# TrevorS/voxtral-mini-realtime-rs

Measured on AMD Instinct MI355X. Metric: decode_tok_per_s, higher is better.
Workload: dtype f32

## Files before the change

### voxtral-mini-realtime-rs_amd/csrc/vox_api.cpp

```cpp
#include "../../include/voxtral_hip.h"
#include "vox_kernels.h"

#include <dlfcn.h>
#include <fcntl.h>
#include <sys/mman.h>
#include <sys/stat.h>
#include <unistd.h>

#include <algorithm>
#include <chrono>
#include <cmath>
#include <cstdarg>
#include <cstdio>
#include <cstdlib>
#include <cstring>
#include <map>
#include <mutex>
#include <string>
#include <unordered_map>
#include <thread>
#include <vector>

using namespace vox;

// ... 661 lines not shown
static std::mutex g_cache_mu; static std::unordered_map<const vox_cache*, uint64_t> g_cache_live; static uint64_t g_cache_gen = 0;
static void cache_register(vox_cache* k) { std::lock_guard<std::mutex> l(g_cache_mu); k->gen = ++g_cache_gen; g_cache_live[k] = k->gen; }
static void cache_unregister(const vox_cache* k) { std::lock_guard<std::mutex> l(g_cache_mu); g_cache_live.erase(k); }
static bool cache_alive(const vox_cache* k, uint64_t gen) { std::lock_guard<std::mutex> l(g_cache_mu); auto it = g_cache_live.find(k); return it != g_cache_live.end() && it->second == gen; }

struct TensorMeta { std::vector<uint64_t> shape; int dtype = 0; uint64_t nbytes = 0; };
struct vox_model {
    vox_ctx* ctx = nullptr; vox_model_cfg cfg{};
    std::vector<vox_model*> twins;
    std::map<std::string, TensorMeta> manifest; bool is_q4 = false;
    uint8_t* arena = nullptr; uint64_t arena_bytes = 0, arena_primary_bytes = 0;
    std::vector<Q4W*> tiled;
    const float *conv1_w = nullptr, *conv1_b = nullptr, *conv2_w = nullptr, *conv2_b = nullptr, *enc_norm = nullptr, *dec_norm = nullptr;
    Q4W conv1_g{}, conv2_g{};
    const float *enc_cos = nullptr, *enc_sin = nullptr, *dec_cos = nullptr, *dec_sin = nullptr;
    int enc_rope_len = 4096, dec_rope_len = 16384;
    std::vector<EncLayer> enc; std::vector<DecLayer> dec; Lin ad0, ad2, tok;
    float* ada_mul = nullptr; bool t_embed_set = false; std::vector<float> t_embed_host;
    float* ws = nullptr; size_t ws_floats = 0;
    float *d_audio = nullptr; int audio_cap = 0;
    float *d_mel = nullptr; size_t mel_cap = 0;
    float *d_samples = nullptr; size_t samples_cap = 0;
    vox_cache* cache = nullptr;
    int *d_tokens = nullptr, *d_pos = nullptr; int tokens_cap = 0;
    float* d_prefix = nullptr;
    float *enc_cos_s = nullptr, *enc_sin_s = nullptr; int enc_rope_s_len = 0;
    int* d_seq_len = nullptr; std::vector<int> h_seq_len;
    int *d_seq_off = nullptr, *d_row_pos = nullptr; size_t row_pos_cap = 0; std::vector<int> h_seq_off, h_row_pos;
    float *d_h = nullptr, *d_q = nullptr, *d_att = nullptr, *d_act = nullptr, *d_logits = nullptr, *d_part_val = nullptr; int* d_part_idx = nullptr;
    float* d_h2 = nullptr; long long* d_wo_acc = nullptr;
    int n_parts = 0, argmax_R = 8;
    bool eng_ok = false, eng_on = true, eng_ready = false; unsigned char* eng_stream = nullptr; unsigned char* eng_state = nullptr; EngLayerTab* eng_tab = nullptr;
    const vox_cache* eng_tab_cache = nullptr; const float* eng_tab_k = nullptr; std::vector<EngLayerTab> eng_tab_host;
    int eng_flags = 128 | 512 | 1, eng_pace = 50;
    unsigned long long eng_launches = 0; unsigned eng_err_host[2] = {0, 0};
    int eng_strikes = 0; bool eng_suspended = false;
    unsigned char* eng_wob = nullptr;
    bool engb_ok = false; unsigned char* engb_state[4] = {nullptr, nullptr, nullptr, nullptr}; EngLayerTab* engb_tab[4] = {nullptr, nullptr, nullptr, nullptr};
    bool engb_on = true; unsigned long long engb_launches = 0; int engb_strikes = 0;
    int batch_sessions = 0;
    int engb_flags = 128 | 1 | 64 | 2048;
    int engb_flags2 = 128 | 1024;
    unsigned engb_err_host[4][2] = {{0, 0}, {0, 0}, {0, 0}, {0, 0}};
    hipGraph_t graph[2] = {nullptr, nullptr}; hipGraphExec_t graph_exec[2] = {nullptr, nullptr}; int graph_unroll = 0, graph_mode = 0;
    const vox_cache* graph_cache = nullptr; const float* graph_audio = nullptr;
    float *pw_x = nullptr, *pw_hidden = nullptr, *pw_logits = nullptr; size_t pw_x_cap = 0, pw_hidden_cap = 0, pw_logits_cap = 0;
    float* pw_part_val = nullptr; int* pw_part_idx = nullptr; int* pw_ids = nullptr; int pw_ids_cap = 0; int* pw_zero = nullptr;
    EngLayerTab* pw_tab = nullptr; const vox_cache* pw_tab_cache = nullptr; uint64_t pw_tab_gen = 0;
    bool pw_memo = false, pw_eng_used = false;
    vox_cache* pw_pend_cache = nullptr; uint64_t pw_pend_gen = 0; int pw_pend_rows = 0; bool pw_verdict_failed = false;
    unsigned* pw_err_pin = nullptr;
    vox_timings timings{};
};

struct Arena {
    uint8_t* base = nullptr; uint64_t off = 0;
    template <class T> T* take(size_t count) {
        off = (off + 255) / 256 * 256;
        T* p = base ? reinterpret_cast<T*>(base + off) : nullptr;
        off += count * sizeof(T);
        return p;
    }
};

#define ENC_PFX "mm_streams_embeddings.embedding_module.whisper_encoder"
#define EMB_PFX "mm_streams_embeddings.embedding_module"
#define TOK_NAME EMB_PFX ".tok_embeddings.weight"
// ... 2553 lines not shown
```

### voxtral-mini-realtime-rs_amd/csrc/vox_engine.hip

```cpp
#include "vox_kernels.h"

#include <hip/hip_fp16.h>

#include <cstdio>
#include <cstdlib>

namespace vox {
namespace {

#include "vox_engine_common.h"

__global__ __launch_bounds__(64) void eng_pack_lm_kernel(Q4W w, unsigned char* __restrict__ stream, size_t op_off, int vocab) {
    const int q = blockIdx.x, b = blockIdx.y, lane = threadIdx.x;
    const int row = lm_rows_per_cu(vocab) * b + q;
    unsigned char* dst = stream + (size_t)NCU * (op_off + (size_t)(q / NCONS) * PK_A) + (size_t)b * PK_A + (size_t)(q % NCONS) * PASS_A;
    const size_t src = (size_t)row * w.nb + lane;
    reinterpret_cast<uint4*>(dst)[lane] = w.qs[src];
    reinterpret_cast<uint16_t*>(dst + PA_S0)[lane] = w.sc[src];
    const size_t sh = (size_t)row * w.nb + 64 + (lane >> 1);
    const uint4 qh = w.qs[sh];
    reinterpret_cast<uint2*>(dst + PA_Q1)[lane] = (lane & 1) ? make_uint2(qh.z, qh.w) : make_uint2(qh.x, qh.y);
    if ((lane & 1) == 0) reinterpret_cast<uint16_t*>(dst + PA_S1)[lane >> 1] = w.sc[sh];
}
__global__ __launch_bounds__(64) void eng_pack_kernel(Q4W w, int op, unsigned char* __restrict__ stream, size_t op_off) {
    const int pk = blockIdx.x / (NCONS * 4), wv = (blockIdx.x / 4) % NCONS, s = blockIdx.x % 4, b = blockIdx.y, lane = threadIdx.x, n = lane & 15, g = lane >> 4;
    const int steps = pk_steps(op, pk); const bool half = pk_half_tile(op, pk);
    if (s >= steps || (half && n >= 8)) return;
    int tile, T; rec_src(op, pk, wv, s, &tile, &T);
    const int row = tile_row(op, b, tile, n), blk0 = step_blk0(op, b, T);
    const size_t pk_bytes = (size_t)op_pk_bytes(op), rec_bytes = half ? REC_H : REC;
    unsigned char* dst = stream + (size_t)NCU * (op_off + (size_t)pk * pk_bytes) + (size_t)b * pk_bytes + (size_t)wv * steps * rec_bytes + (size_t)s * rec_bytes;
    const uint4 q = w.qs[(size_t)row * w.nb + blk0 + (g >> 1)];
    reinterpret_cast<uint2*>(dst)[half ? g * 8 + n : lane] = (g & 1) ? make_uint2(q.z, q.w) : make_uint2(q.x, q.y);
    if (g < 2) reinterpret_cast<uint16_t*>(dst + (half ? REC_H_SC : REC_SC))[(half ? 8 : 16) * g + n] = w.sc[(size_t)row * w.nb + blk0 + g];
}

struct EngCtl {
    unsigned ring_ready[8], ring_done[8];
    unsigned xs0_flag, xs1_flag, xa_flag, qkv_flag;
    unsigned cbar, dead, gathering, gw_flag;
    unsigned xcd_ok, xcc_id, ag_flag, pub_cnt;
    float rstd0, rstd1, pad1, pad2;
    float best_val[16]; int best_idx[16];
    float h_own[16], h1_own[16];
    unsigned ag_done, pad_q[3];
    float rope_c[24], rope_s[24];
};
constexpr int L_RING = 0;
constexpr int L_XS = L_RING + NSLOT * SLOT_BYTES;
constexpr int L_U = L_XS + ED * 4;
constexpr int L_XA = L_U;
constexpr int L_PART = L_U;
constexpr int L_SC = L_U;
constexpr int L_PO = L_SC + SC_MAX * 4;
constexpr int L_PL = L_PO + 12 * 128 * 4;
constexpr int L_QKVN = L_PL + 64;
constexpr int L_TMP = L_QKVN + 384 * 4;
constexpr int L_SSQ = L_TMP + 384 * 4;
constexpr int L_BLK = L_SSQ + NCU * 4;
constexpr int L_TAB = L_BLK + 96 * 8;
constexpr int MAX_LAYERS = 32;
constexpr int L_GW = L_TAB + MAX_LAYERS * (int)sizeof(EngLayerTab);
constexpr int L_CTL = L_GW + (MAX_LAYERS + 1) * 32 * 4;
constexpr int L_TOTAL = L_CTL + (int)sizeof(EngCtl);
static_assert(L_TOTAL <= 160 * 1024, "LDS budget");
static_assert(L_TAB % 16 == 0 && sizeof(EngLayerTab) == 40, "layer table");
static_assert(L_XS % 16 == 0 && L_XA % 16 == 0 && L_QKVN % 16 == 0 && L_PO % 16 == 0 && L_CTL % 16 == 0 && L_BLK % 8 == 0 && 72 * 12 * 4 <= SC_MAX * 4 && 1152 * 4 + 96 * 6 * 4 <= SC_MAX * 4 + 12 * 128 * 4, "aligned carve");

__device__ __forceinline__ void eng_loader(const EngParams& p, EngCtl* c, unsigned ring_lds, int lane, const Tl& tl) {
    Loader<EngCtl, NSLOT> ld; ld.c = c; ld.err = p.err; ld.ring_lds = ring_lds; ld.voff = (unsigned)lane * 16u; ld.thin = (p.flags & 1) != 0; ld.pace = (u64)p.pace_ticks;
    const bool fake = (p.flags & 2) != 0;
    const bool nodma = (p.flags & 32) != 0;
    if (p.flags & 64) ld.pause_ticks = 300;
    if (p.flags & 1024) ld.depth = 2;
    if (p.flags & 2048) ld.depth = 1;
    const u64 base = (u64)p.stream;
    const unsigned n_layer_pk = (unsigned)p.n_layers * PK_LAYER, n_pk = n_layer_pk + (unsigned)lm_packets(p.vocab);
    unsigned l = 0, r = 0;
    u64 off = 0;
#pragma unroll 1
    for (unsigned pk = 0; pk < n_pk; pk++) {
        int bytes = PK_A;
        if (pk < n_layer_pk) {
            if (r < PK_LAYER_M) bytes = PK_M;
            if (r == 0 && (int)l == p.tl_layer) tl(16);
        } else { ld.pace = 0; ld.pause_ticks = 0; ld.depth = 3; }
        const u64 src = fake ? base + (u64)blockIdx.x * PK_A : base + (u64)NCU * off + (u64)blockIdx.x * (u64)bytes;
        if (bytes == PK_M) ld.issue<PK_M>(src, lane, nodma); else ld.issue<PK_A>(src, lane, nodma);
        off += (u64)bytes;
        if (++r == PK_LAYER) { if ((int)l == p.tl_layer) tl(17); r = 0; l++; }
    }
    ld.flush();
    tl(18);
}


__device__ __forceinline__ void comm_probe_x(const EngParams& p, EngCtl* c, int lane, const u64* src, unsigned tag, const Tl& tl, bool T) {
    const srd_t sd = make_srd(src, ED * 8u);
    if (T) tl(20);
    u64 t0 = 0;
    if (p.flags & 512) {
        const u64 tw = wall_clock64();
        while (wall_clock64() - tw < (u64)p.ag_delay_ticks) __builtin_amdgcn_s_sleep(1);
    } else
    for (;;) {
        const u64 gq = ld_gran(sd, 48u * (unsigned)lane);
        if (__all((unsigned)(gq >> 32) == tag)) break;
        if (sweep_bail(t0, tag, c, p.err)) break;
    }
    if (T) tl(21);
}
__device__ __forceinline__ void comm_publish_rows(const EngParams& p, int lane, float hraw, float gw, u64* dst, u64* ssq, unsigned tag, float* own) {
    const int b = blockIdx.x;
    float sq = lane < OWN ? hraw * hraw : 0.f;
    sq = row16_sum_e(sq);
    if (lane < OWN) { publish(dst + OWN * b + lane, tag, hraw * gw); own[lane] = hraw; }
    if (lane == 0) publish(ssq + b, tag, sq);
}

// ... 18 lines not shown
    const unsigned c = own_k >> 5, e = own_k & 31;
    const size_t blk = (size_t)token * (size_t)p.tok_nb + c;
    const unsigned byte = ((const __attribute__((address_space(1))) unsigned char*)(uintptr_t)p.tok_qs)[blk * 16 + (e & 15)];
    const float d = __half2float(__ushort_as_half(((const __attribute__((address_space(1))) unsigned short*)(uintptr_t)p.tok_sc)[blk]));
    const int nib = e < 16 ? (int)(byte & 15u) : (int)(byte >> 4);
    return __fadd_rn(au, __fmul_rn(__fsub_rn((float)nib, 8.0f), d));
}

__device__ __forceinline__ void eng_comm(const EngParams& p, EngCtl* c, unsigned char* lds, const int lane0, const Tl& tl) {
    const int b = blockIdx.x, g = b & 7, j = b >> 3, h = 4 * g + (j >> 3);
    float* xa = reinterpret_cast<float*>(lds + L_XA); float* qkvn = reinterpret_cast<float*>(lds + L_QKVN);
    float* tmp = reinterpret_cast<float*>(lds + L_TMP);
    const EngLayerTab* tab = reinterpret_cast<const EngLayerTab*>(lds + L_TAB);
    const unsigned tag_base = (*p.serial + 1u) * 64u;
    const bool PROBE_SMALL = (p.flags & 4) != 0;
    const int own_r = min(lane0, OWN - 1);
    const unsigned own_k = (unsigned)(OWN * b + own_r);
    const float* gwt = reinterpret_cast<const float*>(lds + L_GW);
    {
        const float g0 = ld_gf(make_srd(p.n_layers > 0 ? tab[0].attn_norm : p.final_norm, ED * 4u), own_k) * (p.n_layers > 0 ? 1.0f : 512.0f);
        const float hraw = (p.flags & ENGF_ARGMAX_IN) ? comm_next_input(p, lane0, own_k) : ld_gf(make_srd(p.h_in, ED * 4u), own_k);
        comm_publish_rows(p, lane0, hraw, g0, p.H0, p.SS0, tag_base, c->h_own);
    }
#pragma unroll 1
    for (int st = 0; st <= 2 * p.n_layers; st++) {
        int lane = lane0; asm volatile("" : "+v"(lane));
        const int l = st >> 1; const bool odd = st & 1, last = st == 2 * p.n_layers, T = l == p.tl_layer;
        const unsigned tag = tag_base + (unsigned)l + 1u;
        if (odd) comm_probe_x(p, c, lane, p.H1, tag, tl, T);
        else comm_probe_x(p, c, lane, p.H0, tag - 1u, tl, false);
        lds_st(&c->gathering, 1u);
        lds_st(&c->ag_flag, (unsigned)st + 1u);
        if (T) tl(odd ? 11 : 8);
        if (p.flags & (1 | 64)) wait_ge(&c->ag_done, NCONS * ((unsigned)st + 1u), c, p.err, ERR_STAGE);
        lds_st(&c->gathering, 0u);
        if (last) break;
        if (!odd) {
            wait_ge(&c->gw_flag, (unsigned)NCONS, c, p.err, ERR_STAGE);
            const bool xloc_nt = (p.flags & 128) != 0 && (p.flags & 4096) != 0 && lds_ld(&c->xcd_ok) != 0;
            {
                wait_ge(&c->pub_cnt, NCONS * (4u * (unsigned)l + 1u), c, p.err, ERR_STAGE);
                lds_st(&c->gathering, 1u);
                float v[6];
                sweep<6>(p.G, (EQD + 2 * EKD) * 8u, tag, [&](int u) { const int i = lane + 64 * u, seg = i >> 7, e = i & 127; return seg == 0 ? 128 * h + e : (seg == 1 ? EQD : EQD + EKD) + 128 * g + e; },
                         [&]() { return lane < 32 ? EQD + 128 * g + 4 * lane : EQD + EKD + 128 * g + 4 * (lane - 32); }, PROBE_SMALL, v, c, p.err, xloc_nt);
                lds_st(&c->gathering, 0u);
#pragma unroll
                for (int u = 0; u < 6; u++) qkvn[lane + 64 * u] = v[u];
                ENG_CFENCE(); lds_st(&c->qkv_flag, (unsigned)l + 1u);
            }
            if (T) tl(9);
            {
                wait_ge(&c->pub_cnt, NCONS * (4u * (unsigned)l + 2u), c, p.err, ERR_STAGE);
                lds_st(&c->gathering, 1u);
                float v[6];
                sweep<6>(p.PW, NPW * ED * 8u, tag, [&](int u) { const int i = lane + 64 * u, hh = i / OWN, r = i - hh * OWN; return hh * ED + OWN * b + r; }, [&]() { return (lane & 31) * ED + OWN * b; }, PROBE_SMALL, v, c, p.err);
#pragma unroll
                for (int u = 0; u < 6; u++) tmp[lane + 64 * u] = v[u];
                lds_st(&c->gathering, 0u);
                ENG_CFENCE();
                float a = 0.f;
                const int r = min(lane, OWN - 1);
#pragma unroll 4
                for (int hh = 0; hh < NPW; hh++) a += tmp[hh * OWN + r];
                wait_ge(&c->gw_flag, (unsigned)NCONS, c, p.err, ERR_STAGE);
                if (!((p.flags & 16384) && blockIdx.x == 7 && l == 1))
                    comm_publish_rows(p, lane, c->h_own[r] + a, gwt[(l * 2 + 1) * 16 + r], p.H1, p.SS1, tag, c->h1_own);
// ... 132 lines not shown
    e = max(e, -100);
    const float f = ldexpf(1.0f, 26 - e);
    int xi[4];
#pragma unroll
    for (int i = 0; i < 4; i++) xi[i] = (int)rintf(v[i] * f);
    int s = (xi[0] + xi[1]) + (xi[2] + xi[3]);
    s += dppi<0xB1>(s); s += dppi<0x4E>(s); s += dppi<0x141>(s);
    if ((lane & 7) == 0) *binfo_blk = make_float2(-8.0f * (float)s, ldexpf(1.0f, e - 26));
    const int e0 = 4 * (lane & 7), h = (e0 >> 3) & 1, off = (e0 & 4) + 8 * (e0 >> 4);
#pragma unroll
    for (int cdig = 0; cdig < 4; cdig++) {
        unsigned d = 0;
#pragma unroll
        for (int i = 0; i < 4; i++) { const int dv = cdig < 3 ? (xi[i] >> (7 * cdig)) & 127 : xi[i] >> 21; d |= (unsigned)(dv & 0xFF) << (8 * i); }
        *reinterpret_cast<unsigned*>(plane_blk + (cdig * 2 + h) * 16 + off) = d;
    }
}

struct Cons {
    const EngParams& p; EngCtl* c; unsigned char* lds; int cw, lane; unsigned P; unsigned cbar_n;
    __device__ __forceinline__ Cons(const EngParams& p_, EngCtl* c_, unsigned char* lds_, int cw_, int lane_) : p(p_), c(c_), lds(lds_), cw(cw_), lane(lane_), P(0), cbar_n(0) {}
    __device__ __forceinline__ void cbarrier() {
        cbar_n += NCONS;
        ENG_CFENCE();
        if (lane == 0) __hip_atomic_fetch_add(&c->cbar, 1u, RLX, WG);
        wait_ge(&c->cbar, cbar_n, c, p.err, ERR_CBAR);
    }
    __device__ __forceinline__ void published(const Tl& tl, int evt) {
        ENG_CFENCE();
        if (lane == 0) { const unsigned old = __hip_atomic_fetch_add(&c->pub_cnt, 1u, RLX, WG); if (evt >= 0 && tl.buf && old % NCONS == NCONS - 1) tl.buf[evt] = wall_clock64(); }
    }
    __device__ __forceinline__ const unsigned char* slot_wait(unsigned pk, int share_bytes, int& slot) {
        slot = (int)(pk % NSLOT); const unsigned k = pk / NSLOT;
        wait_ge(&c->ring_ready[slot], k + 1u, c, p.err, ERR_RING);
        return lds + L_RING + slot * SLOT_BYTES + cw * share_bytes;
    }
    __device__ __forceinline__ void slot_release(int slot) {
        ENG_CFENCE();
        if (lane == 0) __hip_atomic_fetch_add(&c->ring_done[slot], 1u, RLX, WG);
    }
    __device__ __forceinline__ void fetch(unsigned pk, PassA& P_) {
        int slot; const unsigned char* base = slot_wait(pk, PASS_A, slot);
        P_.q0 = reinterpret_cast<const uint4*>(base)[lane];
        P_.q1 = reinterpret_cast<const uint2*>(base + PA_Q1)[lane];
        P_.s0 = __half2float(__ushort_as_half(reinterpret_cast<const unsigned short*>(base + PA_S0)[lane]));
        P_.s1 = __half2float(__ushort_as_half(reinterpret_cast<const unsigned short*>(base + PA_S1)[lane >> 1]));
        slot_release(slot);
    }
    static __device__ __forceinline__ float dot(const PassA& P_, const XA& xr) { return fmaf(P_.s1, half_dot(P_.q1, xr.xh, xr.m8h), P_.s0 * block_dot(P_.q0, xr.x, xr.m8)); }

    template <bool DIGITS>
    __device__ __forceinline__ float all_gather(const u64* src, const u64* ssq, unsigned tag, unsigned stage, unsigned char* xs, float* ssl, float2* binfo, const Tl& tl, bool T) {
        wait_ge(&c->ag_flag, stage + 1u, c, p.err, ERR_STAGE);
        const srd_t sd = make_srd(src, ED * 8u), qd = make_srd(ssq, NCU * 8u);
        int ln = lane; asm volatile("" : "+v"(ln));
        if (DIGITS) {
            const unsigned q = 64u * (unsigned)cw + (unsigned)ln;
            u32x4 ra, rb; u64 rq = 0, t0 = 0;
            for (;;) {
                ra = __builtin_bit_cast(u32x4, __builtin_amdgcn_raw_buffer_load_b128(sd, (int)(q * 32u), 0, 16));
                rb = __builtin_bit_cast(u32x4, __builtin_amdgcn_raw_buffer_load_b128(sd, (int)(q * 32u + 16u), 0, 16));
                if (cw < 4) rq = ld_gran(qd, 64u * (unsigned)cw + (unsigned)ln);
                bool ok = ra.y == tag && ra.w == tag && rb.y == tag && rb.w == tag;
                if (cw < 4) ok &= (unsigned)(rq >> 32) == tag;
                if (__all(ok)) break;
                if (sweep_bail(t0, tag, c, p.err)) break;
            }
            if (T) tl(22);
// ... 79 lines not shown
        if (lane0 == 0) __hip_atomic_fetch_add(&c->gw_flag, 1u, RLX, WG);
    }
    float best = -INFINITY; int best_i = 0x7fffffff;
    bool xloc = false;

#pragma unroll 1
    for (int it = 0; it <= n_items; it++) {
        int lane = lane0; asm volatile("" : "+v"(lane));
        const int l = it / 3, op = it == n_items ? (int)EOP_LM : (it - 3 * l == 0 ? (int)EOP_QKV : it - 3 * l == 1 ? (int)EOP_W13 : (int)EOP_W2);
        const bool T = l == p.tl_layer && cw == 0 && op != EOP_LM;
        const int tlev = l == p.tl_layer ? 1 : 0;
        const unsigned tag = tag_base + (unsigned)l + 1u;
        const EngLayerTab* L = reinterpret_cast<const EngLayerTab*>(lds + L_TAB) + (op == EOP_LM ? 0 : l);
        if (op == EOP_QKV) {
            const gf_p kc = as_g(L->kc) + (size_t)g * p.max_seq * EHD, vc = as_g(L->vc) + (size_t)g * p.max_seq * EHD;
            const int t12 = cw * 64 + lane;
            const int part_ = t12 & 7, ks = t12 >> 3;
            RecR rq[8];
            {
                int s0, s1, s2;
                const unsigned char* b0 = cs.slot_wait(cs.P, 2 * REC, s0);
                rq[0] = rec_read(b0, false, lane); rq[1] = rec_read(b0 + REC, false, lane);
                cs.slot_release(s0);
                const unsigned char* b1 = cs.slot_wait(cs.P + 1, 2 * REC, s1);
                rq[2] = rec_read(b1, false, lane); rq[3] = rec_read(b1 + REC, false, lane);
                cs.slot_release(s1);
                const unsigned char* b2 = cs.slot_wait(cs.P + 2, 4 * REC_H, s2);
#pragma unroll
                for (int i = 0; i < 4; i++) rq[4 + i] = rec_read(b2 + i * REC_H, true, lane);
                cs.slot_release(s2);
                cs.P += QKV_PK;
            }
            cs.all_gather<true>(p.H0, p.SS0, tag - 1u, 2u * (unsigned)l, xs, ssl, binfo, tl, false);
            if (T) tl(0);
            constexpr int NKP = 2;
            float4 kpre[NKP][4];
            auto kload = [&](int u) {
                const unsigned ko = (unsigned)(j_lo + min(ks + 96 * u, last_old)) * EHD + part_ * 16;
#pragma unroll
                for (int e = 0; e < 4; e++) kpre[u][e] = make_float4(0.f, 0.f, 0.f, 0.f);
                if (ks + 96 * u < n_old) {
#pragma unroll
                    for (int e = 0; e < 4; e++) kpre[u][e] = ldg4(kc + (ko + 4 * e));
                }
            };
            kload(0);
            {
                float a0 = 0.f, a1 = 0.f;
#pragma unroll
                for (int i = 0; i < 4; i++) {
                    const StepCtx cx = load_ctx(xs, binfo, 2 * (4 * cw + i), lane);
                    a0 = mstep(rq[i], cx, a0); a1 = mstep(rq[4 + i], cx, a1);
                }
                a0 = g01_sum(a0, lane); a1 = g01_sum(a1, lane);
                if (lane < 16) part[lane * NCONS + cw] = a0;
                if (lane < 8) part[(16 + lane) * NCONS + cw] = a1;
            }
            cs.cbarrier();
            if (it == 0) { wait_ge(&c->gw_flag, (unsigned)NCONS, c, p.err, ERR_STAGE); xloc = (p.flags & 128) != 0 && lds_ld(&c->xcd_ok) != 0; }
            if (cw == 0) {
                const int r = min(lane, 23);
                float a = 0.f;
#pragma unroll
                for (int w = 0; w < NCONS; w++) a += part[r * NCONS + w];
                a *= cs.rstd_staged(ssl);
                const float rc = c->rope_c[r], rs = c->rope_s[r];
                const float o = dppf<0xB1>(a);
                const float y = (lane & 1) ? fmaf(o, rs, a * rc) : fmaf(-o, rs, a * rc);
                if (lane < 24) {
                    const int n = lane < 16 ? 128 * h + 16 * s + lane : lane < 20 ? EQD + 128 * g + 4 * j + (lane - 16) : EQD + EKD + 128 * g + 4 * j + (lane - 20);
                    publish_b(p.G, (EQD + 2 * EKD) * 8u, (unsigned)n, tag, y, xloc);
                    if (lane >= 16) (lane < 20 ? kc : vc)[(size_t)pos * EHD + (n & 127)] = y;
                }
            }
            cs.published(tl, tlev ? 28 : -1);
            if (T) tl(1);
            kload(1);
            float2 vpre[16];
#pragma unroll
            for (int u = 0; u < 16; u++) {
                vpre[u] = make_float2(0.f, 0.f);
                if (cw + 12 * u < n_old) {
                    const fv2 v = *(const __attribute__((address_space(1))) fv2*)(vc + ((unsigned)(j_lo + cw + 12 * u) * EHD + lane * 2));
                    vpre[u] = make_float2(v.x, v.y);
                }
            }
            wait_ge(&c->qkv_flag, (unsigned)l + 1u, c, p.err, ERR_STAGE);
            if (T) tl(2);
            {
                float qv[16];
#pragma unroll
                for (int e = 0; e < 4; e++) { const float4 v = *reinterpret_cast<const float4*>(qkvn + part_ * 16 + 4 * e); qv[4 * e] = v.x; qv[4 * e + 1] = v.y; qv[4 * e + 2] = v.z; qv[4 * e + 3] = v.w; }
                auto dot16 = [&](const float4 (&kk)[4]) {
                    float sacc = 0.f;
#pragma unroll
                    for (int e = 0; e < 4; e++) { sacc = fmaf(qv[4 * e], kk[e].x, sacc); sacc = fmaf(qv[4 * e + 1], kk[e].y, sacc); sacc = fmaf(qv[4 * e + 2], kk[e].z, sacc); sacc = fmaf(qv[4 * e + 3], kk[e].w, sacc); }
                    return group8_sum_e(sacc);
                };
#pragma unroll
                for (int u = 0; u < NKP; u++) {
                    const float sv = dot16(kpre[u]);
                    const int i = ks + 96 * u;
                    if (part_ == 0 && i < n_old) sc[i] = sv * scale;
                }
                for (int i0 = 96 * NKP; i0 < n_old; i0 += 96 * NKP) {
#pragma unroll
                    for (int u = 0; u < NKP; u++) {
                        const int i = i0 + ks + 96 * u;
                        const unsigned ko = (unsigned)(j_lo + min(i, last_old)) * EHD + part_ * 16;
#pragma unroll
                        for (int e = 0; e < 4; e++) kpre[u][e] = make_float4(0.f, 0.f, 0.f, 0.f);
                        if (i < n_old) {
#pragma unroll
                            for (int e = 0; e < 4; e++) kpre[u][e] = ldg4(kc + (ko + 4 * e));
                        }
                    }
#pragma unroll
                    for (int u = 0; u < NKP; u++) {
                        const float sv = dot16(kpre[u]);
                        const int i = i0 + ks + 96 * u;
// ... 45 lines not shown
                    const float pr_ = expf(sc[n_old] - mx); const float2 vv = *reinterpret_cast<const float2*>(qkvn + 256 + lane * 2);
                    o.x = fmaf(pr_, vv.x, o.x); o.y = fmaf(pr_, vv.y, o.y); lsum += pr_;
                }
                po[cw * 64 + lane] = o;
                if (lane == 0) pl[cw] = lsum;
            }
            if (T) tl(23);
            cs.cbarrier();
            if (T) tl(25);
            if (lane < 32) {
                const float4* po4 = reinterpret_cast<const float4*>(po);
                float4 so = make_float4(0.f, 0.f, 0.f, 0.f); float sl = 0.f;
#pragma unroll
                for (int q = 0; q < 12; q++) { const float4 a = po4[q * 32 + lane]; so.x += a.x; so.y += a.y; so.z += a.z; so.w += a.w; sl += pl[q]; }
                const float inv = 1.0f / sl;
                const float v[4] = {so.x * inv, so.y * inv, so.z * inv, so.w * inv};
                to_digits(v, lane, xs + (8 * cw + (lane >> 3)) * 128, binfo + 8 * cw + (lane >> 3));
            }
            if (T) tl(3);
            {
                StepCtx cx[2];
#pragma unroll
                for (int i = 0; i < 2; i++) cx[i] = load_ctx(xs, binfo, 8 * cw + 2 * i, lane);
#pragma unroll
                for (int i = 0; i < WO_PK; i++) {
                    int sl_; const unsigned char* bb = cs.slot_wait(cs.P + i, 2 * REC, sl_);
                    float a = mstep(bb, false, lane, cx[0], 0.f); a = mstep(bb + REC, false, lane, cx[1], a);
                    cs.slot_release(sl_);
                    a = g01_sum(a, lane);
                    if (lane < 16) publish_b(p.PW, NPW * ED * 8u, (unsigned)(h * ED + 384 * s + 16 * (2 * cw + i) + lane), tag, a, false);
                }
                cs.P += WO_PK;
                cs.published(tl, tlev ? 29 : -1);
            }
            if (T) tl(4);
            continue;
        }
        if (op == EOP_W13) {
            constexpr int NPRE = 3;
            RecR rw[4 * NPRE];
#pragma unroll
            for (int ti = 0; ti < NPRE; ti++) {
                int s0, s1;
                const unsigned char* b0 = cs.slot_wait(cs.P + 2 * ti, 2 * REC, s0);
                rw[4 * ti] = rec_read(b0, false, lane); rw[4 * ti + 1] = rec_read(b0 + REC, false, lane);
                cs.slot_release(s0);
                const unsigned char* b1 = cs.slot_wait(cs.P + 2 * ti + 1, 2 * REC, s1);
                rw[4 * ti + 2] = rec_read(b1, false, lane); rw[4 * ti + 3] = rec_read(b1 + REC, false, lane);
                cs.slot_release(s1);
            }
            cs.all_gather<true>(p.H1, p.SS1, tag, 2u * (unsigned)l + 1u, xs, ssl, binfo, tl, T);
            if (T) tl(5);
            StepCtx cx[4];
#pragma unroll
            for (int i = 0; i < 4; i++) cx[i] = load_ctx(xs, binfo, 2 * (4 * cw + i), lane);
            if (T) tl(24);
#pragma unroll
            for (int ti = 0; ti < NPRE; ti++) {
                float a = 0.f;
#pragma unroll
                for (int i = 0; i < 4; i++) a = mstep(rw[4 * ti + i], cx[i], a);
                a = g01_sum(a, lane);
                if (lane < 16) part[(16 * ti + lane) * NCONS + cw] = a;
            }
#pragma unroll 1
            for (int ti = NPRE; ti < 4; ti++) {
                int s0, s1;
                const unsigned char* b0 = cs.slot_wait(cs.P + 2 * ti, 2 * REC, s0);
                const unsigned char* b1 = cs.slot_wait(cs.P + 2 * ti + 1, 2 * REC, s1);
                float a = mstep(b0, false, lane, cx[0], 0.f); a = mstep(b0 + REC, false, lane, cx[1], a);
                a = mstep(b1, false, lane, cx[2], a); a = mstep(b1 + REC, false, lane, cx[3], a);
                cs.slot_release(s0); cs.slot_release(s1);
                a = g01_sum(a, lane);
                if (lane < 16) part[(16 * ti + lane) * NCONS + cw] = a;
            }
            {
                int s2; const unsigned char* b2 = cs.slot_wait(cs.P + 8, 4 * REC_H, s2);
                float a = 0.f;
#pragma unroll
                for (int i = 0; i < 4; i++) a = mstep(b2 + i * REC_H, true, lane, cx[i], a);
                cs.slot_release(s2);
                a = g01_sum(a, lane);
                if (lane < 8) part[(64 + lane) * NCONS + cw] = a;
            }
            cs.P += W13_PK;
            cs.cbarrier();
            if (cw < 2) {
                const int r = min(64 * cw + lane, 71);
                float a = 0.f;
#pragma unroll
                for (int w = 0; w < NCONS; w++) a += part[r * NCONS + w];
                a *= cs.rstd_staged(ssl);
                const float up = dppf<0xB1>(a);
                if ((lane & 1) == 0 && 64 * cw + lane < 72) publish_b(p.A, EF * 8u, (unsigned)(1152 * g + 36 * j + (r >> 1)), tag, silu_e(a) * up, xloc);
            }
            cs.published(tl, tlev ? 30 : -1);
            if (T) tl(6);
            continue;
        }
        if (op == EOP_W2) {
            RecR r2[9];
#pragma unroll
            for (int i = 0; i < W2_PK; i++) {
                int sl_; const unsigned char* bb = cs.slot_wait(cs.P + i, 3 * REC, sl_);
#pragma unroll
                for (int k = 0; k < 3; k++) r2[3 * i + k] = rec_read(bb + k * REC, false, lane);
                cs.slot_release(sl_);
            }
            wait_ge(&c->xa_flag, (unsigned)l + 1u, c, p.err, ERR_STAGE);
            if (T) tl(7);
            const int ksl = cw % 6, tg = cw / 6;
            if (lane < 48) {
                const float4 v4 = *reinterpret_cast<const float4*>(xa + 32 * (6 * ksl + (lane >> 3)) + 4 * (lane & 7));
                const float v[4] = {v4.x, v4.y, v4.z, v4.w};
                to_digits(v, lane, xs + (8 * cw + (lane >> 3)) * 128, binfo + 8 * cw + (lane >> 3));
            }
            StepCtx cx[3];
#pragma unroll
            for (int i = 0; i < 3; i++) cx[i] = load_ctx(xs, binfo, 8 * cw + 2 * i, lane);
#pragma unroll
            for (int i = 0; i < W2_PK; i++) {
                float a = mstep(r2[3 * i], cx[0], 0.f); a = mstep(r2[3 * i + 1], cx[1], a); a = mstep(r2[3 * i + 2], cx[2], a);
                a = g01_sum(a, lane);
                if (lane < 16) part2[(16 * (3 * tg + i) + lane) * 6 + ksl] = a;
            }
            cs.P += W2_PK;
            cs.cbarrier();
            if (cw < 2) {
                const int r = min(64 * cw + lane, 95);
                float a = 0.f;
#pragma unroll
                for (int w = 0; w < 6; w++) a += part2[r * 6 + w];
                if (64 * cw + lane < 96) publish_b(p.P2, NP2 * ED * 8u, (unsigned)(g * ED + 96 * j + r), tag, a, false);
            }
            cs.published(tl, tlev ? 31 : -1);
            if (T) tl(14);
            continue;
        }
        const float rstd = cs.all_gather<false>(p.H0, p.SS0, tag_base + (unsigned)p.n_layers, 2u * (unsigned)p.n_layers, xs, ssl, binfo, tl, false);
        XA xr; xr.load(reinterpret_cast<const float*>(xs), lane, 64 + (lane >> 1), lane & 1);
        const int n_pass = lm_packets(p.vocab);
        PassA Qa, Qb;
        cs.fetch(cs.P, Qa);
#pragma unroll 1
        for (int t = 0; t < n_pass; t++) {
            const int q = cw + NCONS * t;
            if (t + 1 < n_pass) cs.fetch(cs.P + t + 1, Qb);
            if (q < npass_lm) {
                const float r = wave_sum_e(Cons::dot(Qa, xr)) * rstd;
                const int n = row0_lm + q;
                if (p.logits_out && lane == 0) p.logits_out[n] = r;
                if (r > best || (r == best && n < best_i)) { best = r; best_i = n; }
            }
            Qa = Qb;
        }
        cs.P += (unsigned)n_pass;
    }
    if (lane0 == 0) { c->best_val[cw] = best; c->best_idx[cw] = best_i; }
    cs.cbarrier();
    if (cw == 0 && lane0 == 0) {
        float bv = c->best_val[0]; int bi = c->best_idx[0];
        for (int w = 1; w < NCONS; w++) { const float v = c->best_val[w]; const int ii = c->best_idx[w]; if (v > bv || (v == bv && ii < bi)) { bv = v; bi = ii; } }
        p.part_val[b] = bv; p.part_idx[b] = bi;
    }
    if (cw == 0) tl(15);
}

__global__ __launch_bounds__(NTHR, 1) void decode_engine_kernel(const EngParams p) {
// ... 110 lines not shown
```

### voxtral-mini-realtime-rs_amd/csrc/vox_engine_common.h

```cpp
#pragma once

typedef unsigned long long u64;
typedef float f2 __attribute__((ext_vector_type(2)));
typedef unsigned int u32x4 __attribute__((ext_vector_type(4)));

constexpr int ED = 3072, ENH = 32, ENKV = 8, EHD = 128, EQD = ENH * EHD, EKD = ENKV * EHD, EF = 9216;
constexpr int NCU = 256, NCONS = 12, NWAVES = NCONS + 2, NTHR = 64 * NWAVES;
constexpr int REC = 576, REC_H = 288, REC_SC = 512, REC_H_SC = 256;
constexpr int PASS_A = 1728;
constexpr int PA_Q1 = 1024, PA_S0 = 1536, PA_S1 = 1664;
constexpr int PK_A = NCONS * PASS_A, PK_M = NCONS * 2 * REC;
constexpr int LINES_A = (PK_A + 1023) / 1024, LINES_M = (PK_M + 1023) / 1024;
static_assert(LINES_A == 21 && LINES_M == 14, "wait_vmcnt() enumerates the in-flight line counts 14 / 21 / 28 / 35 / 42");
constexpr int SLOT_BYTES = PK_A, NSLOT = 6;
constexpr int QKV_PK = 3, WO_PK = 2, W13_PK = 9, W2_PK = 3, PK_LAYER = QKV_PK + WO_PK + W13_PK + W2_PK, PK_LAYER_M = QKV_PK + WO_PK + W13_PK;
constexpr int LAYER_BYTES = PK_LAYER_M * PK_M + W2_PK * PK_A;
constexpr int OFF_QKV = 0, OFF_WO = QKV_PK * PK_M, OFF_W13 = OFF_WO + WO_PK * PK_M, OFF_W2 = OFF_W13 + W13_PK * PK_M;
static_assert(LAYER_BYTES == 255744, "layer bytes");
constexpr int SC_MAX = 1024;
constexpr int OWN = ED / NCU;
constexpr int NPW = ENH, NP2 = ENKV;
constexpr int NPWB = ENKV;
constexpr size_t WOB_LAYER_BYTES = (size_t)WO_PK * PK_M;
constexpr u64 TIMEOUT_TICKS = 2000000;
// ... 98 lines not shown
    unsigned keep;
    const unsigned lds_dst = (unsigned)__builtin_amdgcn_readfirstlane((int)lds_dst_);
    const u64 gsrc = ((u64)(unsigned)__builtin_amdgcn_readfirstlane((int)(unsigned)(gsrc_ >> 32)) << 32) | (u64)(unsigned)__builtin_amdgcn_readfirstlane((int)(unsigned)gsrc_);
    asm volatile("s_mov_b32 %0, m0\n\ts_mov_b32 m0, %2\n\ts_nop 0\n\tglobal_load_lds_dwordx4 %1, %3 nt\n\ts_mov_b32 m0, %0"
                 : "=&s"(keep) : "v"(voff), "s"(lds_dst), "s"(gsrc) : "memory");
}
__device__ __forceinline__ void dma_lines4(unsigned voff, unsigned lds_dst_, u64 gsrc_) {
    unsigned keep;
    const unsigned lds_dst = (unsigned)__builtin_amdgcn_readfirstlane((int)lds_dst_);
    const u64 gsrc = ((u64)(unsigned)__builtin_amdgcn_readfirstlane((int)(unsigned)(gsrc_ >> 32)) << 32) | (u64)(unsigned)__builtin_amdgcn_readfirstlane((int)(unsigned)gsrc_);
    asm volatile("s_mov_b32 %0, m0\n\ts_mov_b32 m0, %2\n\ts_nop 0\n\tglobal_load_lds_dwordx4 %1, %3 nt\n\tglobal_load_lds_dwordx4 %1, %3 offset:1024 nt\n\t"
                 "global_load_lds_dwordx4 %1, %3 offset:2048 nt\n\tglobal_load_lds_dwordx4 %1, %3 offset:3072 nt\n\ts_mov_b32 m0, %0"
                 : "=&s"(keep) : "v"(voff), "s"(lds_dst), "s"(gsrc) : "memory");
}
__device__ __forceinline__ void wait_vmcnt(int n) {
    switch (n) {
    case 0: asm volatile("s_waitcnt vmcnt(0)" ::: "memory"); break;
    case 14: asm volatile("s_waitcnt vmcnt(14)" ::: "memory"); break;
    case 21: asm volatile("s_waitcnt vmcnt(21)" ::: "memory"); break;
    case 28: asm volatile("s_waitcnt vmcnt(28)" ::: "memory"); break;
    case 35: asm volatile("s_waitcnt vmcnt(35)" ::: "memory"); break;
    case 42: asm volatile("s_waitcnt vmcnt(42)" ::: "memory"); break;
    default: asm volatile("s_waitcnt vmcnt(0)" ::: "memory"); break;
    }
}

template <class Ctl, int NS>
struct Loader {
    Ctl* c; unsigned* err; unsigned ring_lds; unsigned voff;
    int nfl = 0, s0 = 0, l0 = 0, s1 = 0, l1 = 0;
    unsigned P = 0;
    int depth = 3;
    bool thin; u64 pace = 0, t_last = 0, pause_ticks = 0;
    __device__ __forceinline__ void publish_slot(int slot) { lds_st(&c->ring_ready[slot], lds_ld(&c->ring_ready[slot]) + 1u); }
    __device__ __forceinline__ void flush() {
        if (nfl == 2) { wait_vmcnt(l1); publish_slot(s0); s0 = s1; l0 = l1; nfl = 1; }
        if (nfl == 1) { wait_vmcnt(0); publish_slot(s0); nfl = 0; }
    }
    template <int bytes>
    __device__ __forceinline__ void issue(u64 gsrc, int lane, bool nodma) {
        constexpr int full = bytes >> 10, tail = (bytes & 1023) >> 4, lines = full + (tail ? 1 : 0);
        const int slot = (int)(P % NS); const unsigned k = P / NS;
        if (k > 0 && lds_ld(&c->ring_done[slot]) < NCONS * k) {
            flush();
            wait_ge(&c->ring_done[slot], NCONS * k, c, err, ERR_SLOT);
        }
        if (thin && lds_ld(&c->gathering)) flush();
        if (pause_ticks && lds_ld(&c->gathering)) {
            flush();
            const u64 tp = wall_clock64();
            while (lds_ld(&c->gathering) && wall_clock64() - tp < pause_ticks) __builtin_amdgcn_s_sleep(2);
        }
        if (pace) { while (wall_clock64() - t_last < pace) __builtin_amdgcn_s_sleep(1); t_last = wall_clock64(); }
        const unsigned dst = ring_lds + (unsigned)slot * SLOT_BYTES;
        if (!nodma) {
#pragma unroll
            for (int i = 0; i + 4 <= full; i += 4) dma_lines4(voff, dst + (unsigned)i * 1024u, gsrc + (u64)i * 1024u);
#pragma unroll
            for (int i = full & ~3; i < full; i++) dma_line(voff, dst + (unsigned)i * 1024u, gsrc + (u64)i * 1024u);
            if (lane < tail) dma_line(voff, dst + (unsigned)full * 1024u, gsrc + (u64)full * 1024u);
        }
        P++;
        if (nfl == 2) { wait_vmcnt(l1 + lines); publish_slot(s0); s0 = s1; l0 = l1; s1 = slot; l1 = lines; }
        else if (nfl == 1) {
            if (depth <= 2) { wait_vmcnt(lines); publish_slot(s0); s0 = slot; l0 = lines; }
            else { s1 = slot; l1 = lines; nfl = 2; }
        } else { s0 = slot; l0 = lines; nfl = 1; if (depth <= 1) { wait_vmcnt(0); publish_slot(s0); nfl = 0; } }
    }
};

template <class Ctl>
__device__ __forceinline__ bool sweep_bail(u64& t0, unsigned tag, Ctl* c, unsigned* err) {
    __builtin_amdgcn_s_sleep(2);
    if (((++t0) & 31u) != 0) return false;
    if (lds_ld(&c->dead)) return true;
    const u64 t = wall_clock64() << 8;
    if (t0 < 256) t0 = t;
    else if (t - (t0 & ~(u64)255) > (TIMEOUT_TICKS << 8)) {
        lds_st(&c->dead, 1u);
        unsigned ev = (unsigned)ERR_SWEEP | ((unsigned)blockIdx.x << 8) | (tag << 16);
        asm volatile("" : "+s"(ev));
        __hip_atomic_store(err, ev, RLX, AG);
        return true;
    }
    return false;
// ... 33 lines not shown
```

Before: 1438.

## Gate engine weight DMA to compute windows with consumer demand override

Adds a windowed gating mechanism to the persistent decode engine's loader. Weight-packet DMA is issued only while consumer waves are inside compute phases (win counter) and no all-gather is running, or when a consumer is already blocked waiting on a packet (want). A second flag exempts the W13 tail packets from gating. The intent is to cut interference between streaming weight loads and latency-sensitive all-gather and sync phases. The risk is starving the ring and adding stalls, since the loader now flushes and sleeps when the gate is closed, and the all-gather wait also becomes mandatory under the gate flag.

```diff
diff --git a/voxtral-mini-realtime-rs_amd/csrc/vox_api.cpp b/voxtral-mini-realtime-rs_amd/csrc/vox_api.cpp
--- a/voxtral-mini-realtime-rs_amd/csrc/vox_api.cpp
+++ b/voxtral-mini-realtime-rs_amd/csrc/vox_api.cpp
@@ -717,7 +717,7 @@
     int n_parts = 0, argmax_R = 8;
     bool eng_ok = false, eng_on = true, eng_ready = false; unsigned char* eng_stream = nullptr; unsigned char* eng_state = nullptr; EngLayerTab* eng_tab = nullptr;
     const vox_cache* eng_tab_cache = nullptr; const float* eng_tab_k = nullptr; std::vector<EngLayerTab> eng_tab_host;
-    int eng_flags = 128 | 512 | 1, eng_pace = 50;
+    int eng_flags = 128 | 512 | 1 | 8192 | 262144, eng_pace = 50;
     unsigned long long eng_launches = 0; unsigned eng_err_host[2] = {0, 0};
     int eng_strikes = 0; bool eng_suspended = false;
     unsigned char* eng_wob = nullptr;
diff --git a/voxtral-mini-realtime-rs_amd/csrc/vox_engine.hip b/voxtral-mini-realtime-rs_amd/csrc/vox_engine.hip
--- a/voxtral-mini-realtime-rs_amd/csrc/vox_engine.hip
+++ b/voxtral-mini-realtime-rs_amd/csrc/vox_engine.hip
@@ -43,9 +43,11 @@
     float rstd0, rstd1, pad1, pad2;
     float best_val[16]; int best_idx[16];
     float h_own[16], h1_own[16];
-    unsigned ag_done, pad_q[3];
+    unsigned ag_done, win, want, pad_q;
     float rope_c[24], rope_s[24];
 };
+constexpr int ENGF_WIN = 8192, ENGF_W13_TAIL = 262144;
+constexpr int NPRE_W13 = 3;
 constexpr int L_RING = 0;
 constexpr int L_XS = L_RING + NSLOT * SLOT_BYTES;
 constexpr int L_U = L_XS + ED * 4;
@@ -69,6 +71,8 @@
 
 __device__ __forceinline__ void eng_loader(const EngParams& p, EngCtl* c, unsigned ring_lds, int lane, const Tl& tl) {
     Loader<EngCtl, NSLOT> ld; ld.c = c; ld.err = p.err; ld.ring_lds = ring_lds; ld.voff = (unsigned)lane * 16u; ld.thin = (p.flags & 1) != 0; ld.pace = (u64)p.pace_ticks;
+    const bool gated = (p.flags & ENGF_WIN) != 0, tail_free = (p.flags & ENGF_W13_TAIL) != 0;
+    if (gated) ld.want = &c->want;
     const bool fake = (p.flags & 2) != 0;
     const bool nodma = (p.flags & 32) != 0;
     if (p.flags & 64) ld.pause_ticks = 300;
@@ -83,8 +87,9 @@
         int bytes = PK_A;
         if (pk < n_layer_pk) {
             if (r < PK_LAYER_M) bytes = PK_M;
+            ld.win = gated && !(tail_free && r >= QKV_PK + WO_PK + 2 * NPRE_W13 && r < QKV_PK + WO_PK + W13_PK) ? &c->win : nullptr;
             if (r == 0 && (int)l == p.tl_layer) tl(16);
-        } else { ld.pace = 0; ld.pause_ticks = 0; ld.depth = 3; }
+        } else { ld.pace = 0; ld.pause_ticks = 0; ld.depth = 3; ld.win = nullptr; }
         const u64 src = fake ? base + (u64)blockIdx.x * PK_A : base + (u64)NCU * off + (u64)blockIdx.x * (u64)bytes;
         if (bytes == PK_M) ld.issue<PK_M>(src, lane, nodma); else ld.issue<PK_A>(src, lane, nodma);
         off += (u64)bytes;
@@ -169,7 +174,7 @@
         lds_st(&c->gathering, 1u);
         lds_st(&c->ag_flag, (unsigned)st + 1u);
         if (T) tl(odd ? 11 : 8);
-        if (p.flags & (1 | 64)) wait_ge(&c->ag_done, NCONS * ((unsigned)st + 1u), c, p.err, ERR_STAGE);
+        if (p.flags & (1 | 64 | ENGF_WIN)) wait_ge(&c->ag_done, NCONS * ((unsigned)st + 1u), c, p.err, ERR_STAGE);
         lds_st(&c->gathering, 0u);
         if (last) break;
         if (!odd) {
@@ -368,8 +373,14 @@
     }
     __device__ __forceinline__ const unsigned char* slot_wait(unsigned pk, int share_bytes, int& slot) {
         slot = (int)(pk % NSLOT); const unsigned k = pk / NSLOT;
+        if ((p.flags & ENGF_WIN) && lds_ld(&c->ring_ready[slot]) < k + 1u && lane == 0) __hip_atomic_fetch_max(&c->want, pk + 1u, RLX, WG);
         wait_ge(&c->ring_ready[slot], k + 1u, c, p.err, ERR_RING);
         return lds + L_RING + slot * SLOT_BYTES + cw * share_bytes;
+    }
+    __device__ __forceinline__ void window(bool open) {
+        if (!(p.flags & ENGF_WIN)) return;
+        ENG_CFENCE();
+        if (lane == 0) __hip_atomic_fetch_add(&c->win, open ? 1u : ~0u, RLX, WG);
     }
     __device__ __forceinline__ void slot_release(int slot) {
         ENG_CFENCE();
@@ -515,6 +526,7 @@
                 cs.P += QKV_PK;
             }
             cs.all_gather<true>(p.H0, p.SS0, tag - 1u, 2u * (unsigned)l, xs, ssl, binfo, tl, false);
+            cs.window(true);
             if (T) tl(0);
             constexpr int NKP = 2;
             float4 kpre[NKP][4];
@@ -557,6 +569,7 @@
                 }
             }
             cs.published(tl, tlev ? 28 : -1);
+            cs.window(false);
             if (T) tl(1);
             kload(1);
             float2 vpre[16];
@@ -569,6 +582,7 @@
                 }
             }
             wait_ge(&c->qkv_flag, (unsigned)l + 1u, c, p.err, ERR_STAGE);
+            cs.window(true);
             if (T) tl(2);
             {
                 float qv[16];
@@ -680,12 +694,13 @@
                 }
                 cs.P += WO_PK;
                 cs.published(tl, tlev ? 29 : -1);
+                cs.window(false);
             }
             if (T) tl(4);
             continue;
         }
         if (op == EOP_W13) {
-            constexpr int NPRE = 3;
+            constexpr int NPRE = NPRE_W13;
             RecR rw[4 * NPRE];
 #pragma unroll
             for (int ti = 0; ti < NPRE; ti++) {
@@ -698,6 +713,7 @@
                 cs.slot_release(s1);
             }
             cs.all_gather<true>(p.H1, p.SS1, tag, 2u * (unsigned)l + 1u, xs, ssl, binfo, tl, T);
+            cs.window(true);
             if (T) tl(5);
             StepCtx cx[4];
 #pragma unroll
@@ -743,6 +759,7 @@
                 if ((lane & 1) == 0 && 64 * cw + lane < 72) publish_b(p.A, EF * 8u, (unsigned)(1152 * g + 36 * j + (r >> 1)), tag, silu_e(a) * up, xloc);
             }
             cs.published(tl, tlev ? 30 : -1);
+            cs.window(false);
             if (T) tl(6);
             continue;
         }
@@ -756,6 +773,7 @@
                 cs.slot_release(sl_);
             }
             wait_ge(&c->xa_flag, (unsigned)l + 1u, c, p.err, ERR_STAGE);
+            cs.window(true);
             if (T) tl(7);
             const int ksl = cw % 6, tg = cw / 6;
             if (lane < 48) {
@@ -782,6 +800,7 @@
                 if (64 * cw + lane < 96) publish_b(p.P2, NP2 * ED * 8u, (unsigned)(g * ED + 96 * j + r), tag, a, false);
             }
             cs.published(tl, tlev ? 31 : -1);
+            cs.window(false);
             if (T) tl(14);
             continue;
         }
diff --git a/voxtral-mini-realtime-rs_amd/csrc/vox_engine_common.h b/voxtral-mini-realtime-rs_amd/csrc/vox_engine_common.h
--- a/voxtral-mini-realtime-rs_amd/csrc/vox_engine_common.h
+++ b/voxtral-mini-realtime-rs_amd/csrc/vox_engine_common.h
@@ -154,7 +154,19 @@
     unsigned P = 0;
     int depth = 3;
     bool thin; u64 pace = 0, t_last = 0, pause_ticks = 0;
+    const unsigned* win = nullptr; const unsigned* want = nullptr;
     __device__ __forceinline__ void publish_slot(int slot) { lds_st(&c->ring_ready[slot], lds_ld(&c->ring_ready[slot]) + 1u); }
+    __device__ __forceinline__ bool may_issue() const { return lds_ld(want) > P || (lds_ld(win) != 0 && lds_ld(&c->gathering) == 0); }
+    __device__ __forceinline__ void gate() {
+        if (may_issue()) return;
+        flush();
+        const u64 t0 = wall_clock64(); unsigned n = 0;
+        while (!may_issue()) {
+            __builtin_amdgcn_s_sleep(1);
+            if ((++n & 255u) != 0) continue;
+            if (lds_ld(&c->dead) || wall_clock64() - t0 > TIMEOUT_TICKS) break;
+        }
+    }
     __device__ __forceinline__ void flush() {
         if (nfl == 2) { wait_vmcnt(l1); publish_slot(s0); s0 = s1; l0 = l1; nfl = 1; }
         if (nfl == 1) { wait_vmcnt(0); publish_slot(s0); nfl = 0; }
@@ -173,6 +185,7 @@
             const u64 tp = wall_clock64();
             while (lds_ld(&c->gathering) && wall_clock64() - tp < pause_ticks) __builtin_amdgcn_s_sleep(2);
         }
+        if (win) gate();
         if (pace) { while (wall_clock64() - t_last < pace) __builtin_amdgcn_s_sleep(1); t_last = wall_clock64(); }
         const unsigned dst = ring_lds + (unsigned)slot * SLOT_BYTES;
         if (!nodma) {
```

After: 1429 (median of 6 runs). Within noise of the previous version (-0.6%).
